# eryxcoop/acvm-backend-plonky2

Hardware: AMD Instinct MI355X
Metric: prove latency (ms) + proofs/sec at 2^20 LDE rows, 1 GPU(s): value = proofs/sec, witness resident in HBM, 4 proof(s) in flight per GPU; latency_ms_single_proof = lone resident proof; *_host_witness = p2gpu_prove from host RAM (PCIe inside the call) (higher is better)
Workload: dtype u64; 1 GPU; synth(d=17,sha): 131072 gates -> 2^20 LDE rows, 234 wires / 80 routed, KeccakGoldilocksConfig, rate 8, cap 2^4, 28 queries, 16 PoW bits (BASELINE configs[2] shape); degree_bits=17, lde_rows=1048576, mix=sha, public_inputs=0, in_flight_per_gpu=4, proof_bytes=170972

## Files before the change

### acvm-backend-plonky2_amd/csrc/circuit.hpp

```cpp
#pragma once
#include "internal.hpp"
#include "poseidon.hpp"
#include "../../include/p2gpu.h"
#include <cstring>
#include <map>
#include <string>
#include <vector>

#include <exception>

struct p2gpu_circuit;
namespace p2 {

void set_err(const char *fmt, ...);
std::string last_error_copy();
void last_error_restore(const std::string &s);

struct HostHasher {
  int kind = 0;
  const gl_t *prc = nullptr;
};
extern thread_local HostHasher g_hh;
inline size_t hh_bytes() { return g_hh.kind ? 32 : 25; }
inline void sponge_permute(gl_t st[12]) {
// ... 153 lines not shown

struct CircuitState {
  uint32_t d, W, R, NC, num_selectors, K, QF, rate_bits, cap_h, pow_bits, num_queries, n_steps, arity[8];
  uint32_t num_gates, num_pi, flags, PP, nchunks;
  uint32_t hasher = 0;
  size_t n, N;
  uint32_t C;
  std::vector<GateDesc> gates;
  std::vector<gl_t> k_is;
  std::vector<uint8_t> blob_prefix;
  uint32_t nterms = 0, max_gate_constraints = 0;
  uint32_t gate_groups = 1;
  uint32_t half_slots = 0;
  uint32_t gate_groups_half = 1;
  uint32_t sums_groups = 1;
  int half_gates = 1;
  bool half_auto = false;
  gl_t half_cross[16];
  DBuf<gl_t> hsum, htmp_a, htmp_b;
  int device = 0;
  hipStream_t stream = nullptr;
  hipStream_t copy_stream = nullptr;
  std::vector<hipEvent_t> copy_events;
  bool wires_ntt_done = false;
  bool wires_hash_done = false;
  DBuf<uint64_t> hash_state;
  DBuf<uint32_t> wire_nz;
  DBuf<gl_t> wire_scalar;
  uint32_t sparse_row = UINT32_MAX;
  SparseRows sparse_rows;
  DBuf<gl_t> sparse_coeffs, sparse_lde;
  DBuf<gl_t> sparse_partial;
  DBuf<uint32_t> wire_nzlist;
  DBuf<uint32_t> wire_clean;
  int zero_columns = 1;
  bool structured_off = false;
  uint32_t last_dense = 0;
  uint32_t gate_wires = 0;
  int virtual_columns = 1;
  DBuf<gl_t> tw_fwd, tw_inv, scale, inv_scale, d_kis, d_sigmas, fri_scale, qconst;
  DBuf<gl_t> l0_lde;
  DBuf<GateDesc> d_gates;
  DBuf<uint8_t> d_row_gate;
  DBuf<gl_t> d_gconsts, d_prc;
  DBuf<gl_t> d_prc_hash;
  NttPlan *plan_inv = nullptr, *plan_fwd = nullptr;
  std::vector<NttPlan *> fri_plans;
  Batch cs, wires, zp, quot;
  dig_t circuit_digest;
  gl_t poseidon_rc[360];
  gl_t poseidon_rc_gate[360];
  DBuf<gl_t> wires_vals, zp_vals, cp, scan_tmp, apow, qvals, qtmp, pw, partial, ext_apow, f01, f01v, fv;
  std::vector<DBuf<gl_t>> fri_coef, fri_vals;
  std::vector<Batch> fri_trees;
  DBuf<unsigned long long> pow_result;
  PinnedArena pin;
  uint64_t *tail_stage = nullptr;
  DBuf<uint64_t> gather_ptrs;
  DBuf<gl_t> gather_out;
  size_t gather_cap = 0;
  std::vector<uint64_t> h_ptrs;
  std::vector<uint8_t> h_out;
  int shard_rank = 0, shard_world = 1;
  p2gpu_allgather_fn shard_fn = nullptr;
  void *shard_ctx = nullptr;
  void *rccl_comm = nullptr;
  int shard_exercise = 0;
  int shard_zs = 0;
  int shard_reduce = 0;
  int shard_intt = 0;
  DBuf<gl_t> xchg_recv;
  std::vector<p2gpu_circuit *> group;
  struct PeerGroup *peer = nullptr;
  uint64_t pow_hint = UINT64_MAX;
  int profile = 0;
  int self_check = 1;
  int blocking_sync = 0;
  hipEvent_t sync_event = nullptr;
  std::map<std::string, KernelStat> kstats;
  std::vector<PendingEv> pending;
  std::vector<hipEvent_t> event_pool;
};

}

#define P2GPU_CATCH                                                   \
  catch (const std::exception &e) {                                   \
    p2::set_err("internal error: %s", e.what());                      \
    return P2GPU_E_DEVICE;                                            \
  }                                                                   \
  catch (...) {                                                       \
    p2::set_err("internal error");                                    \
    return P2GPU_E_DEVICE;                                            \
  }

struct p2gpu_circuit : p2::CircuitState {};

namespace p2 {
extern void (*g_circuit_release)(p2gpu_circuit *);
void use_hasher(const p2gpu_circuit *c);
void shard_assemble_cap(int world, unsigned rate_bits, size_t cap_per, const dig_t *gathered, std::vector<dig_t> &cap);
int circuit_parse(const uint8_t *blob, size_t len, p2gpu_circuit *c, size_t *off, const uint8_t **cap_in);
const char *gate_validate(uint32_t kind, const uint32_t p[4], uint32_t W, uint32_t gate_consts, uint64_t *wires_used,
                          uint32_t *consts_used);
uint32_t gate_num_constraints(uint32_t kind, const uint32_t p[4]);
uint32_t gate_degree(uint32_t kind, const uint32_t p[4]);
struct BuildPlan {
  size_t n = 0, prefix_len = 0;
  uint32_t R = 0, num_selectors = 0, ngc = 0, NC = 0;
  std::vector<uint32_t> gstart, gend, gsel, arity;
};
int build_plan(const p2gpu_build_params *bp, const p2gpu_gate_decl *gates, uint32_t num_gates, bool have_row_constants, BuildPlan &pl);
int build_prefix(const BuildPlan &pl, const p2gpu_build_params *bp, const p2gpu_gate_decl *gates, uint32_t hasher, uint8_t *out);
bool plonk_identity_holds(const p2gpu_circuit *c, const std::vector<ext_t> &op, const gl_t *betas, const gl_t *gammas,
                          const gl_t *alphas, ext_t zeta, const gl_t pih[4]);
}
```

### acvm-backend-plonky2_amd/csrc/fri.hip

```cpp
#include "internal.hpp"

namespace p2 {

struct ExtSquares {
  ext_t sq[2][32];
};
__global__ __launch_bounds__(256) void ext_powers_bitrev_kernel(ExtSquares S, uint32_t d, gl_t *out0, gl_t *out1) {
  const uint32_t n = 1u << d;
  const uint32_t p = blockIdx.x * blockDim.x + threadIdx.x;
  if (p >= n) return;
  const uint32_t which = blockIdx.y;
  const uint32_t e = bitrev32(p, d);
  ext_t acc = ext_from(1);
  for (uint32_t b = 0; b < d; b++)
    if ((e >> b) & 1) acc = ext_mul(acc, S.sq[which][b]);
  gl_t *out = which ? out1 : out0;
  out[p] = acc.c0;
  out[(size_t)n + p] = acc.c1;
}
void ext_powers_bitrev2(hipStream_t st, ext_t base0, ext_t base1, uint32_t d, gl_t *out0, gl_t *out1) {
  ExtSquares S;
  ext_t a = base0, b = base1;
  for (uint32_t i = 0; i < 32; i++) {
    S.sq[0][i] = a;
// ... 232 lines not shown
    fold[1] = s1[0];
  }
}
void class1_fold(hipStream_t st, const ColHints &h, uint32_t cols, const gl_t *apow, uint32_t j0, gl_t *fold) {
  hipLaunchKernelGGL(class1_fold_kernel, dim3(1), dim3(256), 0, st, h.cls, h.val, cols, apow, j0, fold);
}
void reduce_columns(hipStream_t st, const gl_t *coeffs, uint32_t cols, uint32_t d, const gl_t *apow, uint32_t j0,
                    gl_t *acc, bool accumulate, const uint32_t *nzlist, const gl_t *basis, const gl_t *fold) {
  uint32_t n = 1u << d;
  ProfScope ps("reduce_columns_kernel", 8.0 * (cols + 4.0) * (double)n);
  hipLaunchKernelGGL(reduce_columns_kernel<false>, dim3((n + 63) / 64), dim3(64, 4), 0, st, coeffs, cols, d, apow, j0, acc,
                     accumulate ? 1 : 0, nzlist, basis, fold);
  if (nzlist)
    hipLaunchKernelGGL(reduce_columns_kernel<true>, dim3((n + 63) / 64), dim3(64, 4), 0, st, coeffs, cols, d, apow, j0, acc,
                       accumulate ? 1 : 0, nzlist, basis, fold);
}

__global__ __launch_bounds__(256) void sum_parts_kernel(const gl_t *__restrict__ parts, uint32_t nparts, size_t len, gl_t *__restrict__ out) {
  const size_t p = (size_t)blockIdx.x * blockDim.x + threadIdx.x;
  if (p >= len) return;
  gl_t a = parts[p];
  for (uint32_t q = 1; q < nparts; q++) a = gl_add(a, parts[(size_t)q * len + p]);
  out[p] = a;
}
void sum_parts(hipStream_t st, const gl_t *parts, uint32_t nparts, size_t len, gl_t *out) {
  ProfScope ps("sum_parts_kernel", 8.0 * (nparts + 1.0) * (double)len);
  hipLaunchKernelGGL(sum_parts_kernel, dim3((unsigned)((len + 255) / 256)), dim3(256), 0, st, parts, nparts, len, out);
}

__global__ __launch_bounds__(256) void fri_quotient_values_kernel(const gl_t *F0, const gl_t *F1, uint32_t d,
                                                                  const gl_t *tw, uint32_t tw_shift, ext_t zeta,
                                                                  ext_t gzeta, ext_t f0z, ext_t f1z, ext_t aK,
                                                                  gl_t *out) {
  const uint32_t n = 1u << d;
  const uint32_t k = blockIdx.x * blockDim.x + threadIdx.x;
  if (k >= n) return;
  const uint32_t half = n >> 1;
  gl_t x = d == 0 ? 1 : (k < half ? tw[(size_t)k << tw_shift] : gl_neg(tw[(size_t)(k - half) << tw_shift]));
  ext_t v0 = ext_make(F0[k], F0[(size_t)n + k]), v1 = ext_make(F1[k], F1[(size_t)n + k]);
  ext_t q0 = ext_mul(ext_sub(v0, f0z), ext_inv(ext_sub(ext_from(x), zeta)));
  ext_t q1 = ext_mul(ext_sub(v1, f1z), ext_inv(ext_sub(ext_from(x), gzeta)));
  ext_t r = ext_add(ext_mul(aK, q0), q1);
  out[k] = r.c0;
  out[(size_t)n + k] = r.c1;
}
void fri_quotient_values(hipStream_t st, const gl_t *F0, const gl_t *F1, uint32_t d, const gl_t *tw, uint32_t tw_shift,
                         ext_t zeta, ext_t gzeta, ext_t f0z, ext_t f1z, ext_t aK, gl_t *out) {
  uint32_t n = 1u << d;
  uint32_t threads = n >= 256 ? 256 : 64;
  hipLaunchKernelGGL(fri_quotient_values_kernel, dim3((n + threads - 1) / threads), dim3(threads), 0, st, F0, F1, d, tw,
                     tw_shift, zeta, gzeta, f0z, f1z, aK, out);
}

__global__ __launch_bounds__(256) void fri_fold_kernel(const gl_t *in, uint32_t d, uint32_t ab, ext_t beta, gl_t *out) {
  const uint32_t n = 1u << d, n2 = n >> ab, arity = 1u << ab;
  const uint32_t q = blockIdx.x * blockDim.x + threadIdx.x;
  if (q >= n2) return;
  ext_t acc = ext_from(0);
  for (uint32_t t = arity; t-- > 0;) {
    size_t pos = (size_t)bitrev32(t, ab) * n2 + q;
    acc = ext_add(ext_mul(acc, beta), ext_make(in[pos], in[(size_t)n + pos]));
  }
  out[q] = acc.c0;
  out[(size_t)n2 + q] = acc.c1;
}
void fri_fold(hipStream_t st, const gl_t *in, uint32_t d, uint32_t ab, ext_t beta, gl_t *out) {
  uint32_t n2 = (1u << d) >> ab;
  uint32_t threads = n2 >= 256 ? 256 : 64;
  hipLaunchKernelGGL(fri_fold_kernel, dim3((n2 + threads - 1) / threads), dim3(threads), 0, st, in, d, ab, beta, out);
}

struct PowState {
  gl_t s[12];
};
template <int H>
__global__ __launch_bounds__(256) void pow_kernel(PowState st0, uint32_t pos, uint32_t pow_bits, uint64_t base,
                                                  uint64_t count, unsigned long long *result, const gl_t *__restrict__ prc) {
  const uint64_t i = (uint64_t)blockIdx.x * blockDim.x + threadIdx.x;
  if (i >= count) return;
  const uint64_t w = base + i;
  gl_t st[12];
#pragma unroll
  for (int j = 0; j < 12; j++) st[j] = st0.s[j];
#pragma unroll
  for (int j = 0; j < 12; j++)
    if ((uint32_t)j == pos) st[j] = w;
  if constexpr (H == 1) {
    poseidon_permute_dev(st, prc);
  } else {
    keccak_permutation12<8>(st);
  }
  const uint64_t resp = st[7];
  if (pow_bits == 0 || (resp >> (64 - pow_bits)) == 0) atomicMin(result, (unsigned long long)w);
}
void pow_search(hipStream_t st, const gl_t state[12], uint32_t pos, uint32_t pow_bits, uint64_t base, uint64_t count,
                unsigned long long *result, const gl_t *prc) {
  PowState s;
  for (int i = 0; i < 12; i++) s.s[i] = state[i];
  ProfScope ps("pow_kernel", 0.0);
  if (prc) hipLaunchKernelGGL(pow_kernel<1>, dim3((unsigned)((count + 255) / 256)), dim3(256), 0, st, s, pos, pow_bits, base, count, result, prc);
  else hipLaunchKernelGGL(pow_kernel<0>, dim3((unsigned)((count + 255) / 256)), dim3(256), 0, st, s, pos, pow_bits, base, count, result, prc);
}

__global__ void gather_kernel(const uint64_t *addr, uint32_t count, gl_t *out) {
  uint32_t i = blockIdx.x * blockDim.x + threadIdx.x;
  if (i < count) out[i] = addr[i] ? *(const gl_t *)(uintptr_t)addr[i] : 0;
}
void gather_u64(hipStream_t st, const uint64_t *addr, uint32_t count, gl_t *out) {
  if (!count) return;
  ProfScope ps("gather_kernel", 24.0 * count);
  hipLaunchKernelGGL(gather_kernel, dim3((count + 255) / 256), dim3(256), 0, st, addr, count, out);
}

}
```

### acvm-backend-plonky2_amd/csrc/handle.hip

```cpp
#include "prover_internal.hpp"
#include <functional>

using namespace p2;

namespace {

void release_for_destroy(p2gpu_circuit *c) {
  for (p2gpu_circuit *m : c->group) {
    m->peer = nullptr;
    release_for_destroy(m);
    delete m;
  }
  c->group.clear();
  if (c->peer && c->shard_rank == 0) {
    for (auto e : c->peer->recv_free) if (e) (void)hipEventDestroy(e);
    for (auto e : c->peer->sent) if (e) (void)hipEventDestroy(e);
    delete c->peer;
  }
  c->peer = nullptr;
  (void)hipSetDevice(c->device);
  if (c->stream) (void)hipStreamSynchronize(c->stream);
  if (c->rccl_comm) (void)rccl().CommDestroy((ncclComm_t)c->rccl_comm);
  c->rccl_comm = nullptr;
  circuit_release(c);
// ... 225 lines not shown
  }
  CK(hipMemcpy(c->d_row_gate.p, rg.data(), n, hipMemcpyHostToDevice), "copy row_gate");
  if (ngc)
    CK(hipMemcpy(c->d_gconsts.p, constants + (size_t)c->num_selectors * n, 8 * (size_t)ngc * n, hipMemcpyHostToDevice), "copy gconsts");
  return P2GPU_OK;
}

int alloc_proof_buffers(p2gpu_circuit *c) {
  hipStream_t st = c->stream;
  const size_t n = c->n;
  const uint32_t d = c->d, K = c->K, C = c->C;
  const uint32_t ncs = c->NC + c->R, nzp = K * (1 + c->PP), nq = K * c->QF;
  const uint32_t nall = ncs + c->W + nzp + nq;
  if (batch_alloc(c, c->cs, ncs) || batch_alloc(c, c->wires, c->W) || batch_alloc(c, c->zp, nzp) || batch_alloc(c, c->quot, nq)) return P2GPU_E_DEVICE;
  CK(c->wires_vals.alloc((size_t)c->W * n), "alloc wires");
  CK(c->wire_nz.alloc(c->W), "alloc wire flags");
  CK(c->wire_nzlist.alloc(c->W + 1), "alloc wire flags");
  CK(c->wire_clean.alloc(c->W), "alloc wire flags");
  CK(hipMemsetAsync(c->wire_clean.p, 0, sizeof(uint32_t) * c->W, c->stream), "clear wire flags");
  CK(c->wire_scalar.alloc((size_t)MAX_SPARSE_ROWS * c->W), "alloc wire flags");
  if (c->sparse_row != UINT32_MAX) {
    const uint32_t nr = c->sparse_rows.count;
    CK(c->sparse_coeffs.alloc((size_t)nr * n), "alloc sparse basis");
    CK(c->sparse_lde.alloc((size_t)nr * C * n), "alloc sparse basis");
    CK(c->sparse_partial.alloc(16 * 2 + 2), "alloc sparse basis");
    const gl_t one = 1;
    CK(hipMemsetAsync(c->sparse_coeffs.p, 0, 8 * (size_t)nr * n, st), "sparse basis");
    for (uint32_t s = 0; s < nr; s++)
      CK(hipMemcpyAsync(c->sparse_coeffs.p + (size_t)s * n + c->sparse_rows.row[s], &one, 8, hipMemcpyHostToDevice, st), "sparse basis");
    CK(hipStreamSynchronize(st), "sparse basis");
    ntt_batch(st, c->plan_inv, c->sparse_coeffs.p, c->sparse_coeffs.p, nr, 1, nullptr, gl_inv((gl_t)n), false);
    for (uint32_t s = 0; s < nr; s++)
      ntt_batch(st, c->plan_fwd, c->sparse_coeffs.p + (size_t)s * n, c->sparse_lde.p + (size_t)s * C * n, 1, C, c->scale.p, 1, false);
  }
  CK(c->zp_vals.alloc((size_t)nzp * n), "alloc zp");
  CK(c->cp.alloc((size_t)K * (c->nchunks + 1) * n), "alloc cp");
  CK(c->scan_tmp.alloc((size_t)K * (n + (n + 255) / 256 + 8)), "alloc scan");
  CK(c->apow.alloc((size_t)2 * c->nterms), "alloc apow");
  CK(c->qvals.alloc((size_t)K * C * n), "alloc qvals");
  CK(c->qtmp.alloc((size_t)K * C * n), "alloc qtmp");
  CK(c->pw.alloc((size_t)4 * n), "alloc pw");
  CK(c->partial.alloc(((size_t)(nall + K) + 8) * 16 * 2), "alloc partial");
  CK(c->ext_apow.alloc((size_t)2 * nall), "alloc ext_apow");
  CK(c->f01.alloc((size_t)4 * n), "alloc f01");
  CK(c->f01v.alloc((size_t)4 * n), "alloc f01v");
  CK(c->fv.alloc((size_t)2 * n), "alloc fv");
  c->fri_coef.resize(c->n_steps + 1);
  c->fri_vals.resize(c->n_steps + 1);
  c->fri_trees.resize(c->n_steps);
  size_t gather_words = 0;
  {
    uint32_t ds = d;
    const size_t cap_per = ((size_t)1 << c->cap_h) >> c->rate_bits;
    for (uint32_t s = 0; s <= c->n_steps; s++) {
      c->fri_plans.push_back(s == 0 ? c->plan_fwd : ntt_plan_create(st, ds, NttDir::ToValues));
      if (!c->fri_plans.back()) { set_err("ntt plan allocation failed"); return P2GPU_E_DEVICE; }
      CK(c->fri_coef[s].alloc((size_t)2 << ds), "alloc fri coef");
      if (s < c->n_steps) {
        CK(c->fri_vals[s].alloc((size_t)2 * C << ds), "alloc fri vals");
        uint32_t ab = c->arity[s];
        if (ab < 1 || ab > 4 || ds < ab || (((size_t)1 << ds) >> ab) < cap_per) { set_err("unsupported FRI reduction arity"); return P2GPU_E_BLOB; }
        if (tree_alloc(c->fri_trees[s], C, ((size_t)1 << ds) >> ab, cap_per)) return P2GPU_E_DEVICE;
        gather_words += (2u << ab) + 4 * (size_t)(ds + c->rate_bits);
        ds -= ab;
      }
    }
  }
  gather_words += nall + 4 * 4 * (size_t)(d + c->rate_bits);
  c->gather_cap = gather_words * c->num_queries + 64;
  CK(c->gather_ptrs.alloc(c->gather_cap), "alloc gather");
  CK(c->gather_out.alloc(c->gather_cap), "alloc gather");
  CK(c->pow_result.alloc(1), "alloc pow");
  {
    size_t n_final = n;
    for (uint32_t s = 0; s < c->n_steps; s++) n_final >>= c->arity[s];
    const size_t caps = (size_t)2 * (4 + c->n_steps) * (sizeof(dig_t) << c->cap_h);
    CK(c->pin.alloc(16 * c->gather_cap + 32 * n_final + 16 * (size_t)(nall + K) * 16 + 16 * (size_t)nall + 16 * (size_t)c->nterms +
                    20 * (size_t)c->W + caps + ((size_t)1 << 18)),
       "alloc pinned staging");
  }
  return P2GPU_OK;
}

struct TableSource {
  const gl_t *constants = nullptr, *sigmas = nullptr;
  const BuildInputs *build = nullptr;
};

int commit_constants_sigmas(p2gpu_circuit *c, const TableSource &src) {
  hipStream_t st = c->stream;
  const size_t n = c->n;
  const uint32_t ncs = c->NC + c->R;
  gl_t *stage = c->cs.lde.p;
  if (src.build) {
    build_selector_columns(st, c, stage);
    if (c->NC > c->num_selectors)
      CK(hipMemcpyAsync(stage + (size_t)c->num_selectors * n, c->d_gconsts.p, 8 * (size_t)(c->NC - c->num_selectors) * n, hipMemcpyDeviceToDevice, st),
         "copy constants");
  } else {
    CK(hipMemcpyAsync(stage, src.constants, 8 * (size_t)c->NC * n, hipMemcpyHostToDevice, st), "copy constants");
  }
  CK(hipMemcpyAsync(stage + (size_t)c->NC * n, c->d_sigmas.p, 8 * (size_t)c->R * n, hipMemcpyDeviceToDevice, st), "copy sigmas");
  ntt_batch(st, c->plan_inv, stage, c->cs.coeffs.p, ncs, 1, nullptr, gl_inv((gl_t)n), false);
  return batch_commit_from_coeffs(c, c->cs);
}

int check_cap_and_digest(p2gpu_circuit *c, const uint8_t *cap_in) {
  if (cap_in) {
    for (size_t i = 0; i < c->cs.cap.size(); i++)
      if (memcmp(cap_in + 32 * i, c->cs.cap[i].w, c->hasher ? 32 : 25)) { set_err("constants_sigmas cap mismatch"); return P2GPU_E_CAP_MISMATCH; }
  }
  if (!(c->flags & 1)) {
    std::vector<gl_t> parts;
    for (auto &dg : c->cs.cap) {
      gl_t e[4];
      digest_elems(dg, e);
      parts.insert(parts.end(), e, e + 4);
    }
    std::vector<gl_t> pad(8, 0);
    pad[0] = 1;
    pad[7] = 1;
    dig_t ds = host_hash_no_pad(pad);
    gl_t e[4];
    digest_elems(ds, e);
    parts.insert(parts.end(), e, e + 4);
    parts.push_back(c->d);
    c->circuit_digest = host_hash_no_pad(parts);
  }
  return P2GPU_OK;
}

// ... 260 lines not shown
  if (int rc = ensure_device()) return rc;
  return circuit_make([&](int device, p2gpu_circuit **h) { return circuit_build_one(b, device, h); }, out_c);
} P2GPU_CATCH

int p2gpu_circuit_export_blob(const p2gpu_circuit *cc, uint8_t *out, size_t *len) try {
  if (!cc || !len) return P2GPU_E_ARG;
  if (int rc = prover_handle(cc)) return rc;
  p2gpu_circuit *c = const_cast<p2gpu_circuit *>(cc);
  const size_t n = c->n, nsel = c->num_selectors, ngc = c->NC - c->num_selectors;
  const size_t need = c->blob_prefix.size() + 8 * ((size_t)c->NC + c->R) * n;
  if (!out || *len < need) {
    const bool probe = out == nullptr;
    *len = need;
    if (probe) return P2GPU_OK;
    set_err("blob buffer too small: need %zu bytes", need);
    return P2GPU_E_BUFFER;
  }
  HIP_TRY(hipSetDevice(c->device));
  Scratch S;
  gl_t *sel = S.alloc<gl_t>(nsel * n);
  if (!sel) { set_err("hipMalloc failed"); (void)hipSetDevice(g_device); return P2GPU_E_DEVICE; }
  build_selector_columns(c->stream, c, sel);
  memcpy(out, c->blob_prefix.data(), c->blob_prefix.size());
  uint8_t *q = out + c->blob_prefix.size();
  hipError_t e = hipMemcpyAsync(q, sel, 8 * nsel * n, hipMemcpyDeviceToHost, c->stream);
  if (e == hipSuccess && ngc) e = hipMemcpyAsync(q + 8 * nsel * n, c->d_gconsts.p, 8 * ngc * n, hipMemcpyDeviceToHost, c->stream);
  if (e == hipSuccess) e = hipMemcpyAsync(q + 8 * (size_t)c->NC * n, c->d_sigmas.p, 8 * (size_t)c->R * n, hipMemcpyDeviceToHost, c->stream);
  const hipError_t e2 = hipStreamSynchronize(c->stream);
  (void)hipSetDevice(g_device);
  HIP_TRY(e);
  HIP_TRY(e2);
  *len = need;
  return P2GPU_OK;
} P2GPU_CATCH




int p2gpu_circuit_set(p2gpu_circuit *c, const char *key, uint64_t value) try {
  if (!c || !key) return P2GPU_E_ARG;
  if (int rc = prover_handle(c)) return rc;
  for (p2gpu_circuit *m : c->group)
    if (int rc = p2gpu_circuit_set(m, key, value)) return rc;
  HIP_TRY(hipSetDevice(c->device));
  std::string k(key);
  if (k == "pow_hint") c->pow_hint = value;
  else if (k == "self_check") c->self_check = (int)value;
  else if (k == "shard_exercise") c->shard_exercise = (int)value;
  else if (k == "shard_intt") c->shard_intt = (int)value;
  else if (k == "shard_reduce") c->shard_reduce = (int)value;
  else if (k == "shard_zs") c->shard_zs = (int)value;
  else if (k == "half_gates") c->half_gates = (int)value;
  else if (k == "blocking_sync") c->blocking_sync = (int)value;
  else if (k == "virtual_columns") {
    c->virtual_columns = (int)value;
    if (c->wire_clean.p) HIP_TRY(hipMemsetAsync(c->wire_clean.p, 0, sizeof(uint32_t) * c->W, c->stream));
  }
  else if (k == "zero_columns") {
    c->zero_columns = (int)value;
    c->structured_off = false;
    if (c->wire_clean.p) HIP_TRY(hipMemsetAsync(c->wire_clean.p, 0, sizeof(uint32_t) * c->W, c->stream));
  }
  else if (k == "profile") {
    flush_kstats(c);
    c->profile = (int)value;
    c->kstats.clear();
  } else {
    set_err("unknown knob %s", key);
    return P2GPU_E_ARG;
  }
  return P2GPU_OK;
} P2GPU_CATCH

static int shard_layout(p2gpu_circuit *c, int rank, int world) {
  HIP_TRY(hipSetDevice(c->device));
  if (c->stream) HIP_TRY(hipStreamSynchronize(c->stream));
  if (c->rccl_comm) {
    (void)rccl().CommDestroy((ncclComm_t)c->rccl_comm);
    c->rccl_comm = nullptr;
  }
  c->shard_rank = rank;
  c->shard_world = world;
  c->shard_fn = nullptr;
  c->shard_ctx = nullptr;
  const uint32_t ncl = c->C / (uint32_t)world;
  const size_t cap_per = ((size_t)1 << c->cap_h) >> c->rate_bits;
  CosetMap cm;
  cm.first = (uint32_t)rank;
  cm.stride = (uint32_t)world;
  Batch *bs[3] = {&c->wires, &c->zp, &c->quot};
  for (Batch *b : bs) {
    b->ncl = ncl;
    b->cm = cm;
    tree_layout(*b, ncl, c->n, cap_per);
  }
  if (c->n_steps > 0) {
    Batch &t0 = c->fri_trees[0];
    t0.ncl = ncl;
    t0.cm = cm;
    tree_layout(t0, ncl, c->n >> c->arity[0], cap_per);
  }
  if (c->wire_clean.p) HIP_TRY(hipMemsetAsync(c->wire_clean.p, 0, sizeof(uint32_t) * c->W, c->stream));
  c->xchg_recv.release();
  HIP_TRY(c->xchg_recv.alloc(std::max({(size_t)world * c->gather_cap, (size_t)c->K * c->C * c->n, (size_t)2 * world * c->n}) + 64));
  return P2GPU_OK;
}
// ... 255 lines not shown
```

### acvm-backend-plonky2_amd/csrc/internal.hpp

```cpp
#pragma once
#include <hip/hip_runtime.h>
#include <cstdlib>
#include <vector>
#include "gl.hpp"
#include "keccak.hpp"
#include "gates.hpp"

namespace p2 {

constexpr int MAX_GATES = 64;
constexpr uint32_t MAX_GATE_CONSTRAINTS = 4096;
constexpr uint32_t MAX_ARITY_BITS = 4;
constexpr int MAX_CHALLENGES = 2;
constexpr int MAX_ROUTED = 128;

inline bool env_flag(const char *name, bool dflt) {
  const char *e = getenv(name);
  return e && *e ? *e != '0' : dflt;
}
inline uint64_t env_uint(const char *name, uint64_t dflt) {
  const char *e = getenv(name);
  return e ? strtoull(e, nullptr, 10) : dflt;
}

// ... 110 lines not shown
  const gl_t *k_is;
  const gl_t *tw;
  const gl_t *apow;
  const GateDesc *gates;
  const GateDesc *host_gates;
  gl_t *out;
  uint32_t tw_shift, d, rate_bits, W, R, NC, num_selectors, K, QF, nchunks, PP, num_gates, nterms, has_poseidon;
  uint32_t gate_groups;
  uint32_t gate_groups_half;
  uint32_t use_half;
  uint32_t nsk;
  gl_t *hsum;
  uint32_t coset_first, coset_stride, ncosets;
  gl_t betas[MAX_CHALLENGES], gammas[MAX_CHALLENGES];
  gl_t pi_hash[4];
  const gl_t *qconst;
  gl_t n_inv;
  const gl_t *l0;
};
void quotient_eval(hipStream_t st, const QuotArgs &a);
void gate_sums_eval(hipStream_t st, const QuotArgs &a, uint32_t groups);
void gate_sums_cross(hipStream_t st, const gl_t *in, const gl_t *inv_scale, gl_t *out, uint32_t d, uint32_t cols, const gl_t F[16]);
void fill_l0_table(hipStream_t st, const gl_t *qconst, const gl_t *tw, uint32_t tw_shift, uint32_t d, uint32_t cosets, gl_t n_inv, gl_t *out);
int poseidon_upload_constants();
void quotient_chunks(hipStream_t st, const gl_t *in, const gl_t *inv_scale, gl_t *out, uint32_t d, uint32_t K,
                     uint32_t rate_bits, gl_t w_inv, gl_t gn_inv, gl_t rate_inv, uint32_t world = 1);

void fill_witness(hipStream_t st, gl_t *wires, const uint8_t *row_gate, const GateDesc *gates, const gl_t *gconsts,
                  const gl_t *prc, uint32_t d, uint32_t ngc, uint32_t num_wires);

void ext_powers_bitrev2(hipStream_t st, ext_t base0, ext_t base1, uint32_t d, gl_t *out0, gl_t *out1);
void eval_columns(hipStream_t st, const gl_t *coeffs, uint32_t cols, uint32_t d, const gl_t *pw, uint32_t parts,
                  gl_t *partial , const ColHints *hints = nullptr, const gl_t *basis_partial = nullptr);
struct EvalSegs {
  struct Seg {
    const gl_t *coeffs;
    const gl_t *pw;
    gl_t *partial;
    uint32_t cols;
  } seg[6];
  uint32_t count = 0, hinted = UINT32_MAX;
  const uint32_t *cls = nullptr;
  const gl_t *val = nullptr, *basis_partial = nullptr;
};
void eval_columns_multi(hipStream_t st, const EvalSegs &S, uint32_t d, uint32_t parts, uint32_t col0 = 0, uint32_t ncols = UINT32_MAX);
void reduce_columns(hipStream_t st, const gl_t *coeffs, uint32_t cols, uint32_t d, const gl_t *apow ,
                    uint32_t j0, gl_t *acc, bool accumulate, const uint32_t *nzlist = nullptr, const gl_t *basis = nullptr,
                    const gl_t *fold = nullptr);
void compact_nonzero(hipStream_t st, const uint32_t *flags, uint32_t cols, uint32_t *list);
void sum_parts(hipStream_t st, const gl_t *parts, uint32_t nparts, size_t len, gl_t *out);
void class1_fold(hipStream_t st, const ColHints &h, uint32_t cols, const gl_t *apow, uint32_t j0, gl_t *fold);
void fri_quotient_values(hipStream_t st, const gl_t *F0, const gl_t *F1, uint32_t d, const gl_t *tw, uint32_t tw_shift,
                         ext_t zeta, ext_t gzeta, ext_t f0z, ext_t f1z, ext_t aK, gl_t *out );
void fri_fold(hipStream_t st, const gl_t *in , uint32_t d, uint32_t arity_bits, ext_t beta, gl_t *out);
void pow_search(hipStream_t st, const gl_t state[12], uint32_t pos, uint32_t pow_bits, uint64_t base, uint64_t count,
                unsigned long long *result, const gl_t *prc = nullptr);
void gather_u64(hipStream_t st, const uint64_t *addr, uint32_t count, gl_t *out);

}
```

### acvm-backend-plonky2_amd/csrc/prover.hip

```cpp
#include "prover_internal.hpp"
#include <chrono>

using namespace p2;

namespace {

bool hostprof_on() {
  static const bool on = env_flag("P2GPU_HOSTPROF", false);
  return on;
}

struct Proof {
  const gl_t *wires_dev;
  const uint64_t *pis;
  uint32_t n_pi;
  Challenger ch;
  gl_t pih[4];
  gl_t betas[MAX_CHALLENGES] = {0, 0}, gammas[MAX_CHALLENGES] = {0, 0}, alphas[MAX_CHALLENGES] = {0, 0};
  ext_t zeta;
  Batch *oracles[4];
  std::vector<ext_t> op;
  uint32_t vfirst;
  const uint32_t *h_cls = nullptr;
  const gl_t *h_val = nullptr;
// ... 227 lines not shown
    const uint32_t G = (uint32_t)c->shard_world, cpr = (nall + G - 1) / G;
    const uint32_t c0 = std::min(cpr * (uint32_t)c->shard_rank, nall), c1 = std::min(c0 + cpr, nall);
    bool first = true;
    uint32_t jo = 0;
    for (int o = 0; o < 4; o++) {
      const uint32_t co = P.oracles[o]->cols;
      const uint32_t lo = std::max(c0, jo) - jo, hi = std::min(c1, jo + co) > jo ? std::min(c1, jo + co) - jo : 0;
      if (hi > lo) {
        reduce_columns(st, P.oracles[o]->coeffs.p + (size_t)lo * n, hi - lo, d, c->ext_apow.p, jo + lo, F0, !first);
        first = false;
      }
      jo += co;
    }
    if (first) HIP_TRY(hipMemsetAsync(F0, 0, 16 * n, st));
    if (int rc = shard_allgather(c, F0, c->xchg_recv.p, 16 * n)) return rc;
    sum_parts(st, c->xchg_recv.p, G, 2 * n, F0);
    reduced = true;
  }
  for (int o = reduced ? 4 : 0; o < 4; o++) {
    const bool hw = batch_colnz(c, *P.oracles[o]) != nullptr;
    const bool unit = hw && c->sparse_coeffs.p != nullptr;
    if (unit) class1_fold(st, wire_hints(c, 0, false), c->W, c->ext_apow.p, j0, c->sparse_partial.p + 32);
    reduce_columns(st, P.oracles[o]->coeffs.p, P.oracles[o]->cols, d, c->ext_apow.p, j0, F0, o != 0,
                   hw ? c->wire_nzlist.p : nullptr, unit ? c->sparse_coeffs.p : nullptr, unit ? c->sparse_partial.p + 32 : nullptr);
    j0 += P.oracles[o]->cols;
  }
  reduce_columns(st, c->zp.coeffs.p, K, d, c->ext_apow.p, 0, F1, false);
  ntt_batch(st, c->plan_fwd, c->f01.p, c->f01v.p, 4, 1, nullptr, 1, false);
  fri_quotient_values(st, c->f01v.p, c->f01v.p + 2 * n, d, c->tw_fwd.p, 0, P.zeta, ext_scale(P.zeta, gl_root(d)), f0z, f1z, ext_pow(alpha, K),
                      c->fv.p);
  ntt_batch(st, c->plan_inv, c->fv.p, c->fri_coef[0].p, 2, 1, nullptr, gl_inv((gl_t)n), false);
  if (c->n_steps > 0) {
    ntt_batch(st, c->plan_fwd, c->fri_coef[0].p, c->fri_vals[0].p, 2, c->fri_trees[0].ncl, c->scale.p, 1, false,
              c->fri_trees[0].cm);
  }
  TRACE(c, "fri final poly lde");
  return 0;
}

int self_check(p2gpu_circuit *c, Proof &P) {
  if (c->self_check && !plonk_identity_holds(c, P.op, P.betas, P.gammas, P.alphas, P.zeta, P.pih)) {
    (void)hipStreamSynchronize(c->stream);
    set_err("witness does not satisfy the circuit: the plonk identity fails at zeta (vanishing != Z_H * quotient)");
    return P2GPU_E_UNSATISFIED;
  }
  g_hp.mark("selfcheck");
  return 0;
}

int fri_commit_steps(p2gpu_circuit *c, Proof &P) {
  hipStream_t st = c->stream;
  uint32_t ds = c->d;
  gl_t shift = GL_GEN;
  for (uint32_t s = 0; s < c->n_steps; s++) {
    const uint32_t ab = c->arity[s];
    Batch &tr = c->fri_trees[s];
    hash_fri_leaves(st, c->fri_vals[s].p, ds, tr.ncl, ab, tr.dig.p, hprc(c));
    if (int rc = tree_build(c, tr, ((size_t)1 << ds) >> ab)) return rc;
    P.ch.observe_cap(tr.cap);
    const ext_t beta = P.ch.get_ext();
    fri_fold(st, c->fri_coef[s].p, ds, ab, beta, c->fri_coef[s + 1].p);
    for (uint32_t q = 0; q < ab; q++) shift = gl_sqr(shift);
    ds -= ab;
    if (s + 1 < c->n_steps) {
      fill_coset_scale(st, c->fri_scale.p, shift, gl_root(ds + c->rate_bits), ds, c->C, 1);
      ntt_batch(st, c->fri_plans[s + 1], c->fri_coef[s + 1].p, c->fri_vals[s + 1].p, 2, c->C, c->fri_scale.p, 1, false);
    }
  }
  const size_t n_final = (size_t)1 << ds;
  P.final_poly.resize(n_final);
  gl_t *raw = c->pin.take<gl_t>(2 * n_final);
  if (!raw) return pin_exhausted();
  HIP_TRY(hipMemcpyAsync(raw, c->fri_coef[c->n_steps].p, 16 * n_final, hipMemcpyDeviceToHost, st));
  g_hp.mark("enq(final_poly)");
  if (int rc_ = wait_stream(c)) return rc_;
  g_hp.mark("WAIT(final_poly)");
  for (size_t j = 0; j < n_final; j++) {
    const size_t p = bitrev32((uint32_t)j, ds);
    P.final_poly[j] = ext_make(raw[p], raw[n_final + p]);
  }
  return 0;
}

int grind(p2gpu_circuit *c, Proof &P) {
  P.pow_witness = c->pow_hint;
  if (P.pow_witness != UINT64_MAX) return 0;
  hipStream_t st = c->stream;
  gl_t inter[12];
  memcpy(inter, P.ch.state, sizeof inter);
  for (int i = 0; i < P.ch.n_in; i++) inter[i] = P.ch.in[i];
  uint64_t batch = 1ull << (c->pow_bits + 1 < 20 ? c->pow_bits + 1 : 20);
  const bool split = sharded(c);
  const uint64_t ranks = split ? (uint64_t)c->shard_world : 1;
  unsigned long long *pw = c->pin.take<unsigned long long>(2), *found = split ? c->pin.take<unsigned long long>(ranks) : pw + 1;
  if (!pw || !found) return pin_exhausted();
  for (uint64_t base = 0;; base += batch, batch = batch < (1ull << 22) ? batch * 2 : batch) {
    pw[0] = ~0ull;
    HIP_TRY(hipMemcpyAsync(c->pow_result.p, &pw[0], 8, hipMemcpyHostToDevice, st));
    const uint64_t per = (batch + ranks - 1) / ranks;
    const uint64_t my0 = base + per * (uint64_t)(split ? c->shard_rank : 0);
    const uint64_t myn = my0 >= base + batch ? 0 : std::min(per, base + batch - my0);
    if (myn) pow_search(st, inter, (uint32_t)P.ch.n_in, c->pow_bits, my0, myn, c->pow_result.p, hprc(c));
    const unsigned long long *result = c->pow_result.p;
    if (split) {
      if (int rc = shard_allgather(c, c->pow_result.p, c->xchg_recv.p, 8)) return rc;
      result = (const unsigned long long *)c->xchg_recv.p;
    }
    HIP_TRY(hipMemcpyAsync(found, result, 8 * ranks, hipMemcpyDeviceToHost, st));
    g_hp.mark("enq(pow)");
    if (int rc_ = wait_stream(c)) return rc_;
    g_hp.mark("WAIT(pow)");
    const unsigned long long res = *std::min_element(found, found + ranks);
    if (res != ~0ull) {
      P.pow_witness = res;
      return 0;
    }
    if (base > (1ull << 40)) {
      set_err("proof of work failed");
      return P2GPU_E_DEVICE;
    }
  }
}

void push_path(std::vector<uint64_t> &ptrs, const Batch &b, unsigned lgC, size_t m0, unsigned lgm0, size_t j, bool mine) {
  const size_t levels = b.level_off.size() - 1;
  if (!mine) {
    ptrs.insert(ptrs.end(), 4 * levels, 0);
    return;
  }
  const uint32_t r = bitrev32((uint32_t)(j >> lgm0), lgC), k = bitrev32((uint32_t)(j & (m0 - 1)), lgm0);
  const uint32_t z = (r - b.cm.first) / b.cm.stride;
  size_t m = m0;
  for (size_t l = 0; l < levels; l++, m >>= 1) {
    const size_t sib = (k & (m - 1)) ^ (m >> 1);
    const uint64_t base = (uint64_t)(uintptr_t)(b.dig.p + b.level_off[l] + (size_t)z * m + sib);
    for (int w = 0; w < 4; w++) ptrs.push_back(base + 8 * w);
  }
}

int answer_queries(p2gpu_circuit *c, Proof &P) {
  hipStream_t st = c->stream;
  const uint32_t d = c->d;
  const size_t n = c->n;
  const unsigned lgC = c->rate_bits;
  std::vector<uint64_t> &ptrs = c->h_ptrs;
  ptrs.clear();
  ptrs.reserve(c->gather_cap);
  const int world = c->shard_world, me = c->shard_rank;
  size_t per_query = 0;
  std::vector<std::pair<size_t, uint32_t>> virt_fix;
  for (size_t x : P.qidx) {
    const uint32_t r = bitrev32((uint32_t)(x >> d), lgC), k = bitrev32((uint32_t)(x & (n - 1)), d);
    const bool mine = (int)(r % (uint32_t)world) == me;
    const size_t start = ptrs.size();
    for (int o = 0; o < 4; o++) {
      const Batch &b = *P.oracles[o];
      const uint32_t z = (r - b.cm.first) / b.cm.stride;
      for (uint32_t col = 0; col < b.cols; col++) {
        if (o == 1 && col >= P.vfirst && P.h_cls[col] < 2u) {
          const bool c1 = P.h_cls[col] == 1u && c->sparse_lde.p;
          if (c1) virt_fix.emplace_back(ptrs.size(), col);
          ptrs.push_back(c1 && mine ? (uint64_t)(uintptr_t)(c->sparse_lde.p + (size_t)r * n + k) : 0);
          continue;
        }
        ptrs.push_back(mine ? (uint64_t)(uintptr_t)(b.lde.p + ((size_t)z * b.cols + col) * n + k) : 0);
      }
      push_path(ptrs, b, lgC, n, d, x, mine);
    }
    size_t xi = x;
    uint32_t dcur = d;
    for (uint32_t s = 0; s < c->n_steps; s++) {
      const uint32_t ab = c->arity[s];
      const Batch &tr = c->fri_trees[s];
      const size_t npc = (size_t)1 << dcur, per = npc >> ab;
      const size_t li = xi >> ab;
      const unsigned lgper = dcur - ab;
      const uint32_t rs = bitrev32((uint32_t)(li >> lgper), lgC), kl = bitrev32((uint32_t)(li & (per - 1)), lgper);
      const uint32_t z = (rs - tr.cm.first) / tr.cm.stride;
      const gl_t *v0 = c->fri_vals[s].p + (size_t)z * 2 * npc;
      for (uint32_t t = 0; t < (1u << ab); t++) {
        const size_t kt = (size_t)bitrev32(t, ab) * per + kl;
        ptrs.push_back(mine ? (uint64_t)(uintptr_t)(v0 + kt) : 0);
        ptrs.push_back(mine ? (uint64_t)(uintptr_t)(v0 + npc + kt) : 0);
      }
      push_path(ptrs, tr, lgC, per, lgper, li, mine);
      xi = li;
      dcur -= ab;
    }
    per_query = ptrs.size() - start;
  }
  g_hp.mark("ptrs");
  if (ptrs.size() > c->gather_cap) {
    set_err("internal: gather buffer too small");
    return P2GPU_E_DEVICE;
  }
  gl_t *gathered = c->pin.take<gl_t>(ptrs.size());
  uint64_t *pptrs = c->pin.take<uint64_t>(ptrs.size());
  if (!gathered || !pptrs) return pin_exhausted();
  memcpy(pptrs, ptrs.data(), ptrs.size() * 8);
  HIP_TRY(hipMemcpyAsync(c->gather_ptrs.p, pptrs, ptrs.size() * 8, hipMemcpyHostToDevice, st));
  gather_u64(st, c->gather_ptrs.p, (uint32_t)ptrs.size(), c->gather_out.p);
  g_hp.mark("launch(gather)");
  if (!sharded(c)) {
    HIP_TRY(hipMemcpyAsync(gathered, c->gather_out.p, ptrs.size() * 8, hipMemcpyDeviceToHost, st));
    g_hp.mark("enq(gather)");
    if (int rc_ = wait_stream(c)) return rc_;
    g_hp.mark("WAIT(gather)");
  } else {
    g_hp.mark("enq(gather)");
    if (int rc = shard_allgather(c, c->gather_out.p, c->xchg_recv.p, ptrs.size() * 8)) return rc;
    g_hp.mark("xchg(gather)");
    std::vector<gl_t> all((size_t)world * ptrs.size());
    HIP_TRY(hipMemcpyAsync(all.data(), c->xchg_recv.p, all.size() * 8, hipMemcpyDeviceToHost, st));
    if (int rc_ = wait_stream(c)) return rc_;
    g_hp.mark("WAIT(gather)");
    for (size_t qi = 0; qi < P.qidx.size(); qi++) {
      const uint32_t owner = bitrev32((uint32_t)(P.qidx[qi] >> d), lgC) % (uint32_t)world;
      memcpy(&gathered[qi * per_query], &all[(size_t)owner * ptrs.size() + qi * per_query], per_query * 8);
    }
  }
  for (auto &f : virt_fix) gathered[f.first] = gl_mul(P.h_val[f.second], gathered[f.first]);
  P.gathered = gathered;
  return 0;
}

struct Buf {
  uint8_t *base = nullptr;
  size_t len = 0, cap = 0;
  bool overflow = false;
  void put(const void *p, size_t n) {
    if (len + n > cap) { overflow = true; return; }
    memcpy(base + len, p, n);
    len += n;
  }
  void u64(uint64_t x) { put(&x, 8); }
  void ext(ext_t e) {
    u64(e.c0);
    u64(e.c1);
  }
  void dig(const dig_t &d) { put(d.w, hh_bytes()); }
};

void write_proof(const p2gpu_circuit *c, const Proof &P, Buf &out) {
  const uint32_t K = c->K, nall = committed_cols(c), nzs = c->NC + c->R + c->W + K;
  for (auto &dg : c->wires.cap) out.dig(dg);
  for (auto &dg : c->zp.cap) out.dig(dg);
  for (auto &dg : c->quot.cap) out.dig(dg);
  for (size_t j = 0; j < nzs; j++) out.ext(P.op[j]);
  for (size_t k = 0; k < K; k++) out.ext(P.op[nall + k]);
  for (size_t j = nzs; j < nall; j++) out.ext(P.op[j]);
  for (uint32_t s = 0; s < c->n_steps; s++)
    for (auto &dg : c->fri_trees[s].cap) out.dig(dg);
  size_t g = 0;
  auto put_path = [&](size_t nsib) {
    uint8_t l = (uint8_t)nsib;
    out.put(&l, 1);
    for (size_t i = 0; i < nsib; i++) {
// ... 277 lines not shown
```

Measured before the change: 225.8 proofs/sec.

## Cut FRI tail copies: precompute coset scales, zero-copy pinned writes for fold, PoW, gather

Several small host-device round trips in the FRI tail are removed. Coset scale tables for each FRI step are precomputed once at setup instead of per proof. The last fold kernel writes the final polynomial, already in natural order, straight into pinned host memory. PoW search writes per-block minima to pinned memory instead of doing a memset-style H2D copy plus a D2H readback, and the query gather kernel reads pointers from and writes results to pinned host memory directly, dropping two memcpys. The cost is device access to host memory over PCIe, which is slower per byte but avoids copy launch latency for these small buffers.

```diff
diff --git a/acvm-backend-plonky2_amd/csrc/circuit.hpp b/acvm-backend-plonky2_amd/csrc/circuit.hpp
--- a/acvm-backend-plonky2_amd/csrc/circuit.hpp
+++ b/acvm-backend-plonky2_amd/csrc/circuit.hpp
@@ -229,6 +229,7 @@
   gl_t poseidon_rc_gate[360];
   DBuf<gl_t> wires_vals, zp_vals, cp, scan_tmp, apow, qvals, qtmp, pw, partial, ext_apow, f01, f01v, fv;
   std::vector<DBuf<gl_t>> fri_coef, fri_vals;
+  std::vector<size_t> fri_scale_off;
   std::vector<Batch> fri_trees;
   DBuf<unsigned long long> pow_result;
   PinnedArena pin;
@@ -253,6 +254,7 @@
   int profile = 0;
   int self_check = 1;
   int blocking_sync = 0;
+  int fri_tail_fused = 1;
   hipEvent_t sync_event = nullptr;
   std::map<std::string, KernelStat> kstats;
   std::vector<PendingEv> pending;
diff --git a/acvm-backend-plonky2_amd/csrc/fri.hip b/acvm-backend-plonky2_amd/csrc/fri.hip
--- a/acvm-backend-plonky2_amd/csrc/fri.hip
+++ b/acvm-backend-plonky2_amd/csrc/fri.hip
@@ -308,7 +308,7 @@
                      tw_shift, zeta, gzeta, f0z, f1z, aK, out);
 }
 
-__global__ __launch_bounds__(256) void fri_fold_kernel(const gl_t *in, uint32_t d, uint32_t ab, ext_t beta, gl_t *out) {
+__global__ __launch_bounds__(256) void fri_fold_kernel(const gl_t *in, uint32_t d, uint32_t ab, ext_t beta, gl_t *out, gl_t *natural) {
   const uint32_t n = 1u << d, n2 = n >> ab, arity = 1u << ab;
   const uint32_t q = blockIdx.x * blockDim.x + threadIdx.x;
   if (q >= n2) return;
@@ -319,43 +319,66 @@
   }
   out[q] = acc.c0;
   out[(size_t)n2 + q] = acc.c1;
-}
-void fri_fold(hipStream_t st, const gl_t *in, uint32_t d, uint32_t ab, ext_t beta, gl_t *out) {
+  if (natural != nullptr) {
+    const uint32_t j = bitrev32(q, d - ab);
+    natural[j] = acc.c0;
+    natural[(size_t)n2 + j] = acc.c1;
+  }
+}
+void fri_fold(hipStream_t st, const gl_t *in, uint32_t d, uint32_t ab, ext_t beta, gl_t *out, gl_t *natural) {
   uint32_t n2 = (1u << d) >> ab;
   uint32_t threads = n2 >= 256 ? 256 : 64;
-  hipLaunchKernelGGL(fri_fold_kernel, dim3((n2 + threads - 1) / threads), dim3(threads), 0, st, in, d, ab, beta, out);
+  hipLaunchKernelGGL(fri_fold_kernel, dim3((n2 + threads - 1) / threads), dim3(threads), 0, st, in, d, ab, beta, out, natural);
 }
 
 struct PowState {
   gl_t s[12];
 };
-template <int H>
+template <int H, bool PUB>
 __global__ __launch_bounds__(256) void pow_kernel(PowState st0, uint32_t pos, uint32_t pow_bits, uint64_t base,
                                                   uint64_t count, unsigned long long *result, const gl_t *__restrict__ prc) {
   const uint64_t i = (uint64_t)blockIdx.x * blockDim.x + threadIdx.x;
-  if (i >= count) return;
   const uint64_t w = base + i;
-  gl_t st[12];
-#pragma unroll
-  for (int j = 0; j < 12; j++) st[j] = st0.s[j];
-#pragma unroll
-  for (int j = 0; j < 12; j++)
-    if ((uint32_t)j == pos) st[j] = w;
-  if constexpr (H == 1) {
-    poseidon_permute_dev(st, prc);
+  __shared__ unsigned long long block_min;
+  if constexpr (PUB) {
+    if (threadIdx.x == 0) block_min = ~0ull;
+    __syncthreads();
   } else {
-    keccak_permutation12<8>(st);
-  }
-  const uint64_t resp = st[7];
-  if (pow_bits == 0 || (resp >> (64 - pow_bits)) == 0) atomicMin(result, (unsigned long long)w);
-}
+    if (i >= count) return;
+  }
+  bool hit = false;
+  if (i < count) {
+    gl_t st[12];
+#pragma unroll
+    for (int j = 0; j < 12; j++) st[j] = st0.s[j];
+#pragma unroll
+    for (int j = 0; j < 12; j++)
+      if ((uint32_t)j == pos) st[j] = w;
+    if constexpr (H == 1) {
+      poseidon_permute_dev(st, prc);
+    } else {
+      keccak_permutation12<8>(st);
+    }
+    const uint64_t resp = st[7];
+    hit = pow_bits == 0 || (resp >> (64 - pow_bits)) == 0;
+  }
+  if constexpr (!PUB) {
+    if (hit) atomicMin(result, (unsigned long long)w);
+  } else {
+    if (hit) atomicMin(&block_min, (unsigned long long)w);
+    __syncthreads();
+    if (threadIdx.x == 0) result[blockIdx.x] = block_min;
+  }
+}
+uint32_t pow_search_blocks(uint64_t count) { return (uint32_t)((count + 255) / 256); }
 void pow_search(hipStream_t st, const gl_t state[12], uint32_t pos, uint32_t pow_bits, uint64_t base, uint64_t count,
-                unsigned long long *result, const gl_t *prc) {
+                unsigned long long *result, const gl_t *prc, bool per_block) {
   PowState s;
   for (int i = 0; i < 12; i++) s.s[i] = state[i];
   ProfScope ps("pow_kernel", 0.0);
-  if (prc) hipLaunchKernelGGL(pow_kernel<1>, dim3((unsigned)((count + 255) / 256)), dim3(256), 0, st, s, pos, pow_bits, base, count, result, prc);
-  else hipLaunchKernelGGL(pow_kernel<0>, dim3((unsigned)((count + 255) / 256)), dim3(256), 0, st, s, pos, pow_bits, base, count, result, prc);
+  const dim3 grid(pow_search_blocks(count)), block(256);
+  auto *k = prc ? (per_block ? pow_kernel<1, true> : pow_kernel<1, false>) : (per_block ? pow_kernel<0, true> : pow_kernel<0, false>);
+  hipLaunchKernelGGL(k, grid, block, 0, st, s, pos, pow_bits, base, count, result, prc);
 }
 
 __global__ void gather_kernel(const uint64_t *addr, uint32_t count, gl_t *out) {
diff --git a/acvm-backend-plonky2_amd/csrc/handle.hip b/acvm-backend-plonky2_amd/csrc/handle.hip
--- a/acvm-backend-plonky2_amd/csrc/handle.hip
+++ b/acvm-backend-plonky2_amd/csrc/handle.hip
@@ -301,7 +301,15 @@
   {
     uint32_t ds = d;
     const size_t cap_per = ((size_t)1 << c->cap_h) >> c->rate_bits;
+    gl_t shift = GL_GEN;
+    size_t scale_off = 0;
+    c->fri_scale_off.assign(c->n_steps + 1, 0);
     for (uint32_t s = 0; s <= c->n_steps; s++) {
+      if (s >= 1 && s < c->n_steps) {
+        c->fri_scale_off[s] = scale_off;
+        fill_coset_scale(st, c->fri_scale.p + scale_off, shift, gl_root(ds + c->rate_bits), ds, C, 1);
+        scale_off += (size_t)C << ds;
+      }
       c->fri_plans.push_back(s == 0 ? c->plan_fwd : ntt_plan_create(st, ds, NttDir::ToValues));
       if (!c->fri_plans.back()) { set_err("ntt plan allocation failed"); return P2GPU_E_DEVICE; }
       CK(c->fri_coef[s].alloc((size_t)2 << ds), "alloc fri coef");
@@ -312,6 +320,7 @@
         if (tree_alloc(c->fri_trees[s], C, ((size_t)1 << ds) >> ab, cap_per)) return P2GPU_E_DEVICE;
         gather_words += (2u << ab) + 4 * (size_t)(ds + c->rate_bits);
         ds -= ab;
+        for (uint32_t q = 0; q < ab; q++) shift = gl_sqr(shift);
       }
     }
   }
@@ -325,7 +334,8 @@
     for (uint32_t s = 0; s < c->n_steps; s++) n_final >>= c->arity[s];
     const size_t caps = (size_t)2 * (4 + c->n_steps) * (sizeof(dig_t) << c->cap_h);
     CK(c->pin.alloc(16 * c->gather_cap + 32 * n_final + 16 * (size_t)(nall + K) * 16 + 16 * (size_t)nall + 16 * (size_t)c->nterms +
-                    20 * (size_t)c->W + caps + ((size_t)1 << 18)),
+                    20 * (size_t)c->W + caps + 8 * (size_t)pow_search_blocks(POW_MAX_BATCH) +
+                    ((size_t)1 << 18)),
        "alloc pinned staging");
   }
   return P2GPU_OK;
@@ -692,6 +702,7 @@
   else if (k == "shard_zs") c->shard_zs = (int)value;
   else if (k == "half_gates") c->half_gates = (int)value;
   else if (k == "blocking_sync") c->blocking_sync = (int)value;
+  else if (k == "fri_tail_fused") c->fri_tail_fused = (int)value;
   else if (k == "virtual_columns") {
     c->virtual_columns = (int)value;
     if (c->wire_clean.p) HIP_TRY(hipMemsetAsync(c->wire_clean.p, 0, sizeof(uint32_t) * c->W, c->stream));
diff --git a/acvm-backend-plonky2_amd/csrc/internal.hpp b/acvm-backend-plonky2_amd/csrc/internal.hpp
--- a/acvm-backend-plonky2_amd/csrc/internal.hpp
+++ b/acvm-backend-plonky2_amd/csrc/internal.hpp
@@ -186,9 +186,11 @@
 void class1_fold(hipStream_t st, const ColHints &h, uint32_t cols, const gl_t *apow, uint32_t j0, gl_t *fold);
 void fri_quotient_values(hipStream_t st, const gl_t *F0, const gl_t *F1, uint32_t d, const gl_t *tw, uint32_t tw_shift,
                          ext_t zeta, ext_t gzeta, ext_t f0z, ext_t f1z, ext_t aK, gl_t *out );
-void fri_fold(hipStream_t st, const gl_t *in , uint32_t d, uint32_t arity_bits, ext_t beta, gl_t *out);
+void fri_fold(hipStream_t st, const gl_t *in , uint32_t d, uint32_t arity_bits, ext_t beta, gl_t *out, gl_t *natural = nullptr);
+constexpr uint64_t POW_MAX_BATCH = 1ull << 22;
+uint32_t pow_search_blocks(uint64_t count);
 void pow_search(hipStream_t st, const gl_t state[12], uint32_t pos, uint32_t pow_bits, uint64_t base, uint64_t count,
-                unsigned long long *result, const gl_t *prc = nullptr);
+                unsigned long long *result, const gl_t *prc = nullptr, bool per_block = false);
 void gather_u64(hipStream_t st, const uint64_t *addr, uint32_t count, gl_t *out);
 
 }
diff --git a/acvm-backend-plonky2_amd/csrc/prover.hip b/acvm-backend-plonky2_amd/csrc/prover.hip
--- a/acvm-backend-plonky2_amd/csrc/prover.hip
+++ b/acvm-backend-plonky2_amd/csrc/prover.hip
@@ -303,6 +303,10 @@
   hipStream_t st = c->stream;
   uint32_t ds = c->d;
   gl_t shift = GL_GEN;
+  size_t n_final = c->n;
+  for (uint32_t s = 0; s < c->n_steps; s++) n_final >>= c->arity[s];
+  gl_t *natural = c->fri_tail_fused && c->n_steps > 0 ? c->pin.take<gl_t>(2 * n_final) : nullptr;
+  if (c->fri_tail_fused && c->n_steps > 0 && !natural) return pin_exhausted();
   for (uint32_t s = 0; s < c->n_steps; s++) {
     const uint32_t ab = c->arity[s];
     Batch &tr = c->fri_trees[s];
@@ -310,24 +314,24 @@
     if (int rc = tree_build(c, tr, ((size_t)1 << ds) >> ab)) return rc;
     P.ch.observe_cap(tr.cap);
     const ext_t beta = P.ch.get_ext();
-    fri_fold(st, c->fri_coef[s].p, ds, ab, beta, c->fri_coef[s + 1].p);
+    fri_fold(st, c->fri_coef[s].p, ds, ab, beta, c->fri_coef[s + 1].p, s + 1 == c->n_steps ? natural : nullptr);
     for (uint32_t q = 0; q < ab; q++) shift = gl_sqr(shift);
     ds -= ab;
     if (s + 1 < c->n_steps) {
-      fill_coset_scale(st, c->fri_scale.p, shift, gl_root(ds + c->rate_bits), ds, c->C, 1);
-      ntt_batch(st, c->fri_plans[s + 1], c->fri_coef[s + 1].p, c->fri_vals[s + 1].p, 2, c->C, c->fri_scale.p, 1, false);
-    }
-  }
-  const size_t n_final = (size_t)1 << ds;
+      gl_t *scale = c->fri_scale.p + c->fri_scale_off[s + 1];
+      if (!c->fri_tail_fused) fill_coset_scale(st, scale, shift, gl_root(ds + c->rate_bits), ds, c->C, 1);
+      ntt_batch(st, c->fri_plans[s + 1], c->fri_coef[s + 1].p, c->fri_vals[s + 1].p, 2, c->C, scale, 1, false);
+    }
+  }
   P.final_poly.resize(n_final);
-  gl_t *raw = c->pin.take<gl_t>(2 * n_final);
+  gl_t *raw = natural ? natural : c->pin.take<gl_t>(2 * n_final);
   if (!raw) return pin_exhausted();
-  HIP_TRY(hipMemcpyAsync(raw, c->fri_coef[c->n_steps].p, 16 * n_final, hipMemcpyDeviceToHost, st));
+  if (!natural) HIP_TRY(hipMemcpyAsync(raw, c->fri_coef[c->n_steps].p, 16 * n_final, hipMemcpyDeviceToHost, st));
   g_hp.mark("enq(final_poly)");
   if (int rc_ = wait_stream(c)) return rc_;
   g_hp.mark("WAIT(final_poly)");
   for (size_t j = 0; j < n_final; j++) {
-    const size_t p = bitrev32((uint32_t)j, ds);
+    const size_t p = natural ? j : bitrev32((uint32_t)j, ds);
     P.final_poly[j] = ext_make(raw[p], raw[n_final + p]);
   }
   return 0;
@@ -345,22 +349,33 @@
   const uint64_t ranks = split ? (uint64_t)c->shard_world : 1;
   unsigned long long *pw = c->pin.take<unsigned long long>(2), *found = split ? c->pin.take<unsigned long long>(ranks) : pw + 1;
   if (!pw || !found) return pin_exhausted();
-  for (uint64_t base = 0;; base += batch, batch = batch < (1ull << 22) ? batch * 2 : batch) {
-    pw[0] = ~0ull;
-    HIP_TRY(hipMemcpyAsync(c->pow_result.p, &pw[0], 8, hipMemcpyHostToDevice, st));
-    const uint64_t per = (batch + ranks - 1) / ranks;
-    const uint64_t my0 = base + per * (uint64_t)(split ? c->shard_rank : 0);
-    const uint64_t myn = my0 >= base + batch ? 0 : std::min(per, base + batch - my0);
-    if (myn) pow_search(st, inter, (uint32_t)P.ch.n_in, c->pow_bits, my0, myn, c->pow_result.p, hprc(c));
-    const unsigned long long *result = c->pow_result.p;
-    if (split) {
-      if (int rc = shard_allgather(c, c->pow_result.p, c->xchg_recv.p, 8)) return rc;
-      result = (const unsigned long long *)c->xchg_recv.p;
-    }
-    HIP_TRY(hipMemcpyAsync(found, result, 8 * ranks, hipMemcpyDeviceToHost, st));
-    g_hp.mark("enq(pow)");
-    if (int rc_ = wait_stream(c)) return rc_;
-    g_hp.mark("WAIT(pow)");
+  const bool per_block = c->fri_tail_fused && !split;
+  unsigned long long *mins = per_block ? c->pin.take<unsigned long long>(pow_search_blocks(POW_MAX_BATCH)) : nullptr;
+  if (per_block && !mins) return pin_exhausted();
+  for (uint64_t base = 0;; base += batch, batch = batch < POW_MAX_BATCH ? batch * 2 : batch) {
+    if (per_block) {
+      pow_search(st, inter, (uint32_t)P.ch.n_in, c->pow_bits, base, batch, mins, hprc(c), true);
+      g_hp.mark("enq(pow)");
+      if (int rc_ = wait_stream(c)) return rc_;
+      g_hp.mark("WAIT(pow)");
+      *found = *std::min_element(mins, mins + pow_search_blocks(batch));
+    } else {
+      pw[0] = ~0ull;
+      HIP_TRY(hipMemcpyAsync(c->pow_result.p, &pw[0], 8, hipMemcpyHostToDevice, st));
+      const uint64_t per = (batch + ranks - 1) / ranks;
+      const uint64_t my0 = base + per * (uint64_t)(split ? c->shard_rank : 0);
+      const uint64_t myn = my0 >= base + batch ? 0 : std::min(per, base + batch - my0);
+      if (myn) pow_search(st, inter, (uint32_t)P.ch.n_in, c->pow_bits, my0, myn, c->pow_result.p, hprc(c));
+      const unsigned long long *result = c->pow_result.p;
+      if (split) {
+        if (int rc = shard_allgather(c, c->pow_result.p, c->xchg_recv.p, 8)) return rc;
+        result = (const unsigned long long *)c->xchg_recv.p;
+      }
+      HIP_TRY(hipMemcpyAsync(found, result, 8 * ranks, hipMemcpyDeviceToHost, st));
+      g_hp.mark("enq(pow)");
+      if (int rc_ = wait_stream(c)) return rc_;
+      g_hp.mark("WAIT(pow)");
+    }
     const unsigned long long res = *std::min_element(found, found + ranks);
     if (res != ~0ull) {
       P.pow_witness = res;
@@ -449,11 +464,16 @@
   uint64_t *pptrs = c->pin.take<uint64_t>(ptrs.size());
   if (!gathered || !pptrs) return pin_exhausted();
   memcpy(pptrs, ptrs.data(), ptrs.size() * 8);
-  HIP_TRY(hipMemcpyAsync(c->gather_ptrs.p, pptrs, ptrs.size() * 8, hipMemcpyHostToDevice, st));
-  gather_u64(st, c->gather_ptrs.p, (uint32_t)ptrs.size(), c->gather_out.p);
+  const bool direct = c->fri_tail_fused && !sharded(c);
+  if (direct) {
+    gather_u64(st, pptrs, (uint32_t)ptrs.size(), gathered);
+  } else {
+    HIP_TRY(hipMemcpyAsync(c->gather_ptrs.p, pptrs, ptrs.size() * 8, hipMemcpyHostToDevice, st));
+    gather_u64(st, c->gather_ptrs.p, (uint32_t)ptrs.size(), c->gather_out.p);
+  }
   g_hp.mark("launch(gather)");
   if (!sharded(c)) {
-    HIP_TRY(hipMemcpyAsync(gathered, c->gather_out.p, ptrs.size() * 8, hipMemcpyDeviceToHost, st));
+    if (!direct) HIP_TRY(hipMemcpyAsync(gathered, c->gather_out.p, ptrs.size() * 8, hipMemcpyDeviceToHost, st));
     g_hp.mark("enq(gather)");
     if (int rc_ = wait_stream(c)) return rc_;
     g_hp.mark("WAIT(gather)");
```

New measurement: 226.2 proofs/sec (median of 2 runs). Within noise of the previous version (+0.2%).
